# leohuang2013/pyannote-audio_speaker-diarization_cpp

Hardware: AMD Instinct MI355X
Metric: real-time factor (audio-sec/wall-sec), 1 h 16 kHz mono per GPU (higher is better)
Workload: dtype f32

## Files before the change

pyannote-audio_speaker-diarization_cpp_amd/csrc/api.cpp:

```cpp
#include "common.h"
#include <algorithm>
#include <cmath>
#include <cstdlib>
#include <fstream>
#include <tuple>

static std::string g_create_err;

int seg_prec(const sd_ctx* c) { return c->seg_precision >= 0 ? c->seg_precision : (c->ecapa_precision != 0 ? 3 : 0); }

extern "C" const char* sd_create_error(void) { return g_create_err.c_str(); }
extern "C" const char* sd_last_error(const sd_ctx* c) { return c ? c->err.c_str() : "null context"; }

extern "C" sd_ctx* sd_create(const char* seg_path, const char* emb_path, int device)
{
    g_create_err.clear();
    int ndev = 0;
    if (hipGetDeviceCount(&ndev) != hipSuccess || ndev <= 0) { g_create_err = "no HIP device available (libsdhip has no CPU fallback)"; return nullptr; }
    if (device < 0 || device >= ndev) { g_create_err = "device id out of range"; return nullptr; }
    if (hipSetDevice(device) != hipSuccess) { g_create_err = "hipSetDevice failed"; return nullptr; }
    sd_ctx* c = new sd_ctx();
    c->device = device;
    hipDeviceProp_t prop;
    if (hipGetDeviceProperties(&prop, device) == hipSuccess) c->num_cu = prop.multiProcessorCount;
// ... 46 lines not shown
    }
    c->pending.clear();
}

extern "C" int sd_kernel_stats(const sd_ctx* cc, const char* kernel, double* total_ms, int64_t* launches, double* flops, double* bytes)
{
    sd_ctx* c = const_cast<sd_ctx*>(cc);
    if (!c || !kernel) return SD_ERR_ARG;
    (void)hipStreamSynchronize(c->stream);
    sd_flush_profile(c);
    auto it = c->stats.find(kernel);
    KernelStat s; if (it != c->stats.end()) s = it->second;
    if (total_ms) *total_ms = s.ms; if (launches) *launches = s.launches; if (flops) *flops = s.flops; if (bytes) *bytes = s.bytes;
    return SD_OK;
}
extern "C" int sd_debug_read_ws(sd_ctx* c, const char* name, int64_t offset, void* h_out, int64_t bytes)
{
    if (!c || !name || !h_out || offset < 0 || bytes < 0) return SD_ERR_ARG;
    auto it = c->ws.find(name);
    if (it == c->ws.end() || !it->second.p) SD_FAIL(c, SD_ERR_ARG, "no workspace named %s", name);
    if ((size_t)(offset + bytes) > it->second.cap) SD_FAIL(c, SD_ERR_ARG, "workspace %s holds %zu bytes", name, it->second.cap);
    HIPCHK(c, hipStreamSynchronize(c->stream));
    HIPCHK(c, hipMemcpy(h_out, (const char*)it->second.p + offset, (size_t)bytes, hipMemcpyDeviceToHost));
    return SD_OK;
}
extern "C" void sd_reset_stats(sd_ctx* c) { if (!c) return; (void)hipStreamSynchronize(c->stream); sd_flush_profile(c); c->stats.clear(); }
extern "C" int sd_stage_ms(const sd_ctx* c, double* ms4) { if (!c || !ms4) return SD_ERR_ARG; for (int i = 0; i < 4; ++i) ms4[i] = c->stage_ms[i]; return SD_OK; }
extern "C" int sd_set_option(sd_ctx* c, const char* key, int64_t v)
{
    if (!c || !key) return SD_ERR_ARG;
    std::string k(key);
    if (k == "emb_batch_items") { c->emb_batch_items = v; c->emb_batch_explicit = true; }
    else if (k == "seg_batch_chunks") c->seg_batch_chunks = v;
    else if (k == "ws_limit_mb") g_ws_limit.store(v > 0 ? (size_t)v << 20 : 0);
    else if (k == "emb_batch_default") { c->emb_batch_items = 3072; c->emb_batch_explicit = false; c->embed_calls = v; }
    else if (k == "linkage_wgs") c->linkage_wgs = v;
    else if (k == "linkage_threads") c->linkage_threads = v;
    else if (k == "linkage_kernel") c->linkage_kernel = v;
    else if (k == "linkage_tie_kernel") c->linkage_tie_kernel = v;
    else if (k == "linkage_zero_phase") c->linkage_zero_phase = v;
    else if (k == "linkage_force_heap") c->linkage_force_heap = v != 0;
    else if (k == "linkage_hx_wide") c->linkage_hx_wide = v != 0;
    else if (k == "linkage_prefetch") c->linkage_prefetch = v != 0;
    else if (k == "linkage_one_xcd") c->linkage_one_xcd = v;
    else if (k == "linkage_square") c->linkage_square = v;
    else if (k == "skip_dead_rows") c->skip_dead_rows = v != 0;
    else if (k == "conv_h256") c->conv_h256 = v != 0;
    else if (k == "conv_glds") c->conv_glds = v != 0;
    else if (k == "conv_pp") c->conv_pp = v != 0;
    else if (k == "conv_glds_f32") c->conv_glds_f32 = v != 0;
    else if (k == "conv_mfma16") { if (v < 0 || v > 2) return SD_ERR_ARG; c->conv_mfma16 = (int)v; }
    else if (k == "conv_rot") { if (v < 0 || v > 3) return SD_ERR_ARG; c->conv_rot = (int)v; }
    else if (k == "conv_stagger") { if (v < 0 || v > 2) return SD_ERR_ARG; c->conv_stagger = (int)v; }
    else if (k == "conv_w256_f32") c->conv_w256_f32 = v != 0;
    else if (k == "conv_pn") c->conv_pn = (int)v;
    else if (k == "ecapa_ld_pad") { if (v < 0 || v > 1024 || ((int64_t)v & 7)) return SD_ERR_ARG; c->ecapa_ld_pad = (int)v; }
    else if (k == "seg_shared_conv0") c->seg_shared_conv0 = v != 0;
    else if (k == "seg_wide_ih") c->seg_wide_ih = v != 0;
    else if (k == "conv_w256_kmin") c->conv_w256_kmin = (int)v;
    else if (k == "conv_pn128") c->conv_pn128 = (int)v;
    else if (k == "seg_precision") { if (v != 0 && v != 3 && v != -1) SD_FAIL(c, SD_ERR_ARG, "seg_precision must be 0 (f32), 3 (split fp16 operands for the LSTM) or -1 (auto: 3 whenever ecapa_precision is not 0)"); c->seg_precision = (int)v; }
    else if (k == "ecapa_precision") { if (v < 0 || v > 3) SD_FAIL(c, SD_ERR_ARG, "ecapa_precision must be 0 (f32), 1 (fp16), 2 (fp16, hi + lo weight planes) or 3 (f32 tensors, split fp16 operands on the wide layers)");
                                        if (hipSetDevice(c->device) != hipSuccess) SD_FAIL(c, SD_ERR_HIP, "hipSetDevice failed");
                                        const int rcw = ensure_ecapa_mode_weights(c, (int)v); if (rcw) return rcw;
                                        c->ecapa_precision = (int)v; }
    else if (k == "ecapa_f16_hp") { if (v != 0 && v != 1 && v != 3) SD_FAIL(c, SD_ERR_ARG, "ecapa_f16_hp must be 0, 1 (MFA output in f32) or 3 (+ the attention branch)"); c->ecapa_f16_hp = (int)v; }
// ... 474 lines not shown
```

pyannote-audio_speaker-diarization_cpp_amd/csrc/common.h:

```cpp
#pragma once
#include <hip/hip_runtime.h>
#include <atomic>
#include <chrono>
#include <cstdint>
#include <cstdio>
#include <cstring>
#include <map>
#include <set>
#include <string>
#include <functional>
#include <initializer_list>
#include <vector>
#include "../../include/sdhip_test.h"

#define SD_T 501
#define SD_TP 501
#define SD_NBINS 201
#define SD_NMELS 80
#define SD_FEAT_LD 96

#define SD_WAV_PAD 512
struct DevWav {
    const float* p;
    int64_t n;
// ... 96 lines not shown
    void* lstm_hh_x[4][2] = {};
    float lstm_hh_inv[4][2] = {};
    ConvLayer lin0, lin1;
    float* cls_w = nullptr; float* cls_b = nullptr;
};

struct StepStash {
    bool clustered = false;
    int64_t N = 0; int K = 0;
    std::vector<int> clusters, cluster_res, hard_pre;
    std::vector<double> X, Xn, soft;
    int64_t ar0 = 0, cr0 = 0, rows = 0, crow_all = 0, nact = 0;
    int64_t infer_items = 0;
};

struct sd_ctx {
    int device = 0;
    hipStream_t stream = nullptr;
    std::string err;
    EcapaWeights ew;
    SegWeights sw;
    std::vector<void*> owned;
    char* warena_cur = nullptr; size_t warena_left = 0;
    std::map<std::string, DevBuf> ws;
    std::set<std::string> rs_taps_filled;
    std::map<std::string, KernelStat> stats;
    bool profile = false;
    bool profile_detail = false;
    std::vector<std::tuple<std::string, hipEvent_t, hipEvent_t, double, double>> pending;
    double stage_ms[4] = {0, 0, 0, 0};
    int64_t emb_batch_items = 3072;
    bool emb_batch_explicit = false;
    int64_t embed_calls = 0;
    int64_t seg_batch_chunks = 4096;
    int num_clusters = -1, min_clusters = -1, max_clusters = -1;
    int ecapa_precision = 0;
    int seg_precision = -1;
    bool ecapa_keep_cat = false;
    int ecapa_f16_hp = 0;
    bool conv_w256_f32 = true;
    int conv_pn128 = 0;
    int ecapa_ld_pad = 0;
    bool seg_wide_ih = true;
    bool seg_shared_conv0 = true;
    int conv_w256_kmin = 0;
    int conv_pn = 0;
    bool conv_h256 = true;
    int conv_mfma16 = 1;
    int conv_rot = 3;
    int conv_stagger = 0;
    bool conv_glds_f32 = false;
    bool conv_pp = true;
    bool conv_glds = true;
    bool skip_dead_rows = true;
    int64_t linkage_wgs = -1;
    int64_t linkage_square = -1;
    int64_t linkage_one_xcd = 1;
    int64_t linkage_zero_phase = 1;
    int64_t linkage_tie_kernel = 1;
    int64_t linkage_prefetch = 0;
    bool linkage_hx_wide = false;
    bool linkage_force_heap = false;
    int64_t linkage_kernel = -1;
    int64_t linkage_threads = 0;
    int num_cu = 256;
    bool constrained_assignment = false;
    int clustering_method = SD_LINKAGE_CENTROID;
// ... 107 lines not shown
float lstm_whh_split(const float* whh , _Float16* planes );
void* weight_alloc(sd_ctx* c, size_t bytes);
int ensure_ecapa_mode_weights(sd_ctx* c, int ecapa_precision);
inline size_t conv_w16_bytes(const ConvLayer& L) { return (size_t)2 * L.KT * L.Cout * L.CinPad16 * 2; }
inline size_t conv_w16x_bytes(const ConvLayer& L) { return (size_t)2 * L.KT * L.Cout * L.CinPad * 2; }
int build_conv_w16(sd_ctx* c, ConvLayer& L, void* d);
int build_conv_w16x(sd_ctx* c, ConvLayer& L, void* d, unsigned* d_max);
int frontend_prepare(sd_ctx* c, const float* d_masks, int64_t items, int64_t first_item, float* d_wav_lens, int* d_nnorm, int* d_nvalid,
                     int* d_flags, bool compact, int* h_n_active, int* d_cidx, std::vector<int>* h_nvalid = nullptr);
int frontend_features(sd_ctx* c, const DevWav& w, int64_t first_item, int64_t run_items, bool compact, const int* d_nnorm,
                      const int* d_rowoff, float* d_feats , bool sig_mode = false);
int frontend_prepare_signals(sd_ctx* c, int64_t items);
#define EC_SPACES 4
struct EcapaRowPlan {
    int64_t n = 0;
    std::vector<int> off[EC_SPACES];
    const int* d_off = nullptr;
};
int ecapa_need_rows(int nvalid, bool skip_dead_rows);
int ecapa_build_rowtab(sd_ctx* c, const int* d_off_out, int base_out, const int* d_off_in, int base_in, int64_t items, int2* d_rowtab);
int ecapa_rows_to_half(sd_ctx* c, const float* d_f32, void* d_f16, int64_t n4);
int ecapa_row_plan(sd_ctx* c, const int* h_nvalid, int64_t n, EcapaRowPlan& plan, int* d_off );
int run_ecapa(sd_ctx* c, const float* d_feats, const int* d_nvalid , const EcapaRowPlan& plan, int64_t a0, int64_t a1, float* d_emb );
std::vector<int64_t> ecapa_plan_batches(const EcapaRowPlan& plan, int64_t cap_rows, bool balance);
int64_t ecapa_round_items(int64_t nb);
int ecapa_run_items(sd_ctx* c, const float* d_feats, const int* d_nvalid, const EcapaRowPlan& plan, int64_t nb, bool balance, float* d_emb);
int run_embed(sd_ctx* c, const DevWav& w, const float* d_masks, int64_t items, int64_t first_item, float* d_emb);
int run_segment(sd_ctx* c, const DevWav& w, int64_t chunk_lo, int64_t chunk_hi, float* d_seg);
int run_segment_rows(sd_ctx* c, const DevWav& rows, int T, float* d_seg, int* frames);
int launch_chunk_norm(sd_ctx* c, const float* d_wav, int64_t origin, int64_t first_chunk, int64_t hop, int L, int64_t chunks, float w, float b, float* xn);
int launch_chunk_stats(sd_ctx* c, const float* d_wav, int64_t origin, int64_t first_chunk, int L, int64_t chunks, float w, float b, float2* st);
int launch_pool_norm(sd_ctx* c, int stage, const float* in, int64_t chunks, int Lc, const float* gw, const float* gb, float* out,
                     const float2* cst, const float* wsum, int chunk_rows);
int launch_lstm_rec(sd_ctx* c, const float* G, const float* whh_f, const float* whh_b, const void* whx_f, const void* whx_b, float inv_f, float inv_b,
                    float* H, int64_t B, int F);
int launch_classifier(sd_ctx* c, const float* y, const float* W, const float* bias, float* seg, int64_t chunks, int F);
__global__ void k_pcm_to_f32(const int16_t* __restrict__ pcm, float* __restrict__ dst, int64_t n);
int pcm_to_wav(sd_ctx* c, const int16_t* d_pcm, int64_t n, DevWav* out);
int f32_to_wav(sd_ctx* c, const float* h_wav, int64_t n, DevWav* out);
inline void clear_stage_ms(sd_ctx* c) { for (double& ms : c->stage_ms) ms = 0; }
int shard_infer(sd_ctx* c, const DevWav& w, int64_t lo, int64_t hi, float* d_seg, float* d_emb, bool seg_done = false);
int finalize(sd_ctx* c, const float* d_seg, const float* d_emb, int64_t chunks, int64_t n, std::vector<sd_turn>& v);
int turns_out(sd_ctx* c, const std::vector<sd_turn>& v, sd_turn** turns, int64_t* n_turns);
int resample_dev(sd_ctx* c, const float* d_in, int64_t n, int32_t in_sr, int32_t out_sr, float* d_out, int64_t n_out);
int run_postseg(sd_ctx* c, const float* d_seg, int64_t chunks, uint8_t* d_bin, float* d_masks, int* d_nact);
int run_count(sd_ctx* c, const uint8_t* d_bin, int64_t chunks, int32_t* d_count, int64_t n_count, double* d_avg = nullptr);
int write_step_dumps(sd_ctx* c, const float* d_seg, const float* d_emb, int64_t chunks, int64_t n_samples, const std::vector<int>& hard_post, int K);
int64_t count_frames_host(int64_t chunks);
int sd_np_rint_host(double v);
int64_t closest_frame_host(double w_start, double w_step, double w_dur, double t);
int run_linkage(sd_ctx* c, const double* d_X, int64_t N, int d, double* d_Z, int method = SD_LINKAGE_CENTROID, int metric = SD_METRIC_EUCLIDEAN);
int run_cluster_labels(sd_ctx* c, const double* d_X, int64_t N, int d, double cutoff, std::vector<int>& labels1, std::vector<double>* Zout = nullptr,
                       int method = SD_LINKAGE_CENTROID, int metric = SD_METRIC_EUCLIDEAN);
int run_clustering(sd_ctx* c, const double* d_emb , int64_t M, int d, std::vector<int>& hard, int* K,
                   int num_clusters = -1, int min_clusters = -1, int max_clusters = -1, std::vector<double>* soft_best = nullptr);
void fcluster_host(const std::vector<double>& Z, int64_t n, double cutoff, std::vector<int>& T);
int64_t activity_frames_host(int64_t chunks);
int64_t activity_rows_host(int64_t nf, int64_t n_samples);
int run_activity_scores(sd_ctx* c, const float* d_seg, int64_t chunks, int kind, double* d_scores, int64_t nf);
int run_activity_regions(sd_ctx* c, const double* d_scores, int64_t rows, int label, std::vector<sd_turn>& turns);
int check_spans(sd_ctx* c, const sd_turn* spans, int64_t n_spans, const char* who);
void spans_to_samples(const sd_turn* spans, int64_t n_spans, int32_t label, int64_t n, std::vector<int64_t>& out);
int run_span_masks(sd_ctx* c, const std::vector<int64_t>& spans, int64_t chunks, int64_t n, float* d_masks );
int run_voiceprint_mean(sd_ctx* c, const float* d_emb , int64_t chunks, double* h_mean , int64_t* n_live);
int run_speaker_dist(sd_ctx* c, const double* d_cen, int64_t K, const double* d_gal, int64_t M, int d, double* d_dist, double* h_dist );
int run_reconstruct(sd_ctx* c, const float* d_seg, const int* d_nact, const int* d_hard, const int32_t* d_count,
// ... 2 lines not shown
```

pyannote-audio_speaker-diarization_cpp_amd/csrc/pyannet.hip:

```cpp
#include "common.h"

typedef float f32x16 __attribute__((ext_vector_type(16)));

__global__ __launch_bounds__(256) void k_chunk_norm(const float* __restrict__ wav, int64_t origin, int64_t first_chunk, int64_t hop, int L,
                                                    float w, float b, float* __restrict__ xn)
{
    __shared__ float red[256];
    const int ck = blockIdx.x, tid = threadIdx.x;
    const int64_t base = (first_chunk + ck) * hop - origin;
    const float* x = wav + base;
    float s = 0.0f;
    for (int j = tid; j < L; j += 256) s += x[j];
    red[tid] = s;
    __syncthreads();
    for (int o = 128; o > 0; o >>= 1) { if (tid < o) red[tid] += red[tid + o]; __syncthreads(); }
    const float mean = red[0] / (float)L;
    __syncthreads();
    float v = 0.0f;
    for (int j = tid; j < L; j += 256) { const float d = x[j] - mean; v += d * d; }
    red[tid] = v;
    __syncthreads();
    for (int o = 128; o > 0; o >>= 1) { if (tid < o) red[tid] += red[tid + o]; __syncthreads(); }
    const float rstd = rsqrtf(red[0] / (float)L + 1e-5f);
    const float a = rstd * w, c = b - mean * rstd * w;
// ... 241 lines not shown
        const float giv[8] = {gi[0].x, gi[0].y, gi[0].z, gi[0].w, gi[1].x, gi[1].y, gi[1].z, gi[1].w};
        const float gfv[8] = {gf[0].x, gf[0].y, gf[0].z, gf[0].w, gf[1].x, gf[1].y, gf[1].z, gf[1].w};
        const float ggv[8] = {gg[0].x, gg[0].y, gg[0].z, gg[0].w, gg[1].x, gg[1].y, gg[1].z, gg[1].w};
        const float gov[8] = {go[0].x, go[0].y, go[0].z, go[0].w, go[1].x, go[1].y, go[1].z, go[1].w};
        float hv[8];
#pragma unroll
        for (int r = 0; r < 8; ++r) {
            const float ig = sigm(acc0[r] * inv + giv[r]);
            const float fg = sigm(acc0[r + 8] * inv + gfv[r]);
            const float gt = tanh_fast(acc1[r] * inv + ggv[r]);
            const float og = sigm(acc1[r + 8] * inv + gov[r]);
            cst[r] = fg * cst[r] + ig * gt;
            hv[r] = og * tanh_fast(cst[r]);
        }
        _Float16* hn = &hbuf[cur ^ 1][li * HXLD];
        lhalf4 h0, l0, h1, l1;
#pragma unroll
        for (int e = 0; e < 4; ++e) {
            h0[e] = (_Float16)hv[e];     l0[e] = (_Float16)(hv[e] - (float)h0[e]);
            h1[e] = (_Float16)hv[4 + e]; l1[e] = (_Float16)(hv[4 + e] - (float)h1[e]);
        }
        *(lhalf4*)(hn + ua) = h0; *(lhalf4*)(hn + 128 + ua) = l0;
        *(lhalf4*)(hn + ub) = h1; *(lhalf4*)(hn + 128 + ub) = l1;
        if (live) {
            float* ho = H + ((size_t)(b0 + li) * F + t) * 256 + dir * 128;
            *(float4*)(ho + ua) = make_float4(hv[0], hv[1], hv[2], hv[3]);
            *(float4*)(ho + ub) = make_float4(hv[4], hv[5], hv[6], hv[7]);
        }
        __syncthreads();
        cur ^= 1;
    }
}

__global__ __launch_bounds__(256) void k_classifier(const float* __restrict__ y, const float* __restrict__ W, const float* __restrict__ bias,
                                                    float* __restrict__ seg, int64_t chunks, int F)
{
    __shared__ float w[3 * 128];
    for (int i = threadIdx.x; i < 384; i += 256) w[i] = W[i];
    __syncthreads();
    const int64_t idx = (int64_t)blockIdx.x * 256 + threadIdx.x;
    if (idx >= chunks * SD_FRAMES) return;
    const int64_t ck = idx / SD_FRAMES;
    const int f = (int)(idx - ck * SD_FRAMES);
    float o0 = 0.0f, o1 = 0.0f, o2 = 0.0f;
    if (f < F) {
        const float* x = y + ((size_t)ck * F + f) * 128;
        float a0 = bias[0], a1 = bias[1], a2 = bias[2];
        for (int k = 0; k < 128; k += 4) {
            const float4 v = *(const float4*)(x + k);
            a0 += v.x * w[k] + v.y * w[k + 1] + v.z * w[k + 2] + v.w * w[k + 3];
            a1 += v.x * w[128 + k] + v.y * w[129 + k] + v.z * w[130 + k] + v.w * w[131 + k];
            a2 += v.x * w[256 + k] + v.y * w[257 + k] + v.z * w[258 + k] + v.w * w[259 + k];
        }
        o0 = 1.0f / (1.0f + expf(-a0)); o1 = 1.0f / (1.0f + expf(-a1)); o2 = 1.0f / (1.0f + expf(-a2));
    }
    seg[idx * 3 + 0] = o0; seg[idx * 3 + 1] = o1; seg[idx * 3 + 2] = o2;
}

__global__ void k_zero_f32(float* p, int64_t n)
{
    const int64_t i = (int64_t)blockIdx.x * blockDim.x + threadIdx.x;
    if (i < n) p[i] = 0.0f;
}

__global__ void k_dense_rowtab(int2* __restrict__ rowtab, int64_t M)
{
// ... 2 lines not shown
}

int launch_chunk_norm(sd_ctx* c, const float* d_wav, int64_t origin, int64_t first_chunk, int64_t hop, int L, int64_t chunks, float w, float b, float* xn)
{
    hipLaunchKernelGGL(k_chunk_norm, dim3((unsigned)chunks), dim3(256), 0, c->stream, d_wav, origin, first_chunk, hop, L, w, b, xn);
    KCHECK(c);
    return SD_OK;
}

int launch_chunk_stats(sd_ctx* c, const float* d_wav, int64_t origin, int64_t first_chunk, int L, int64_t chunks, float w, float b, float2* st)
{
    hipLaunchKernelGGL(k_chunk_stats, dim3((unsigned)chunks), dim3(256), 0, c->stream, d_wav, origin, first_chunk, L, w, b, st);
    KCHECK(c);
    return SD_OK;
}

int launch_pool_norm(sd_ctx* c, int stage, const float* in, int64_t chunks, int Lc, const float* gw, const float* gb, float* out,
                     const float2* cst, const float* wsum, int chunk_rows)
{
    const int Lp = Lc / 3;
    const dim3 grid((unsigned)chunks), block(PN_T);
    if (stage == 0 && cst)
        hipLaunchKernelGGL((k_pool_norm<80, 96, true, true>), grid, block, 0, c->stream, in, Lc, Lp, gw, gb, out, cst, wsum, chunk_rows);
    else if (stage == 0)
        hipLaunchKernelGGL((k_pool_norm<80, 96, true, false>), grid, block, 0, c->stream, in, Lc, Lp, gw, gb, out, nullptr, nullptr, 0);
    else if ((stage == 1 || stage == 2) && !cst)
        hipLaunchKernelGGL((k_pool_norm<60, 64, false, false>), grid, block, 0, c->stream, in, Lc, Lp, gw, gb, out, nullptr, nullptr, 0);
    else
        SD_FAIL(c, SD_ERR_ARG, "k_pool_norm: stage %d%s", stage, cst ? " (shared form)" : "");
    KCHECK(c);
    return SD_OK;
}

int launch_lstm_rec(sd_ctx* c, const float* G, const float* whh_f, const float* whh_b, const void* whx_f, const void* whx_b, float inv_f, float inv_b,
                    float* H, int64_t B, int F)
{
    ProfScope ps(c, "lstm_rec", 2.0 * B * F * 2 * 512 * 128, 0);
    const dim3 grid((unsigned)((B + 31) / 32), 2), block(512);
    if (whx_f && whx_b)
        hipLaunchKernelGGL(k_lstm_rec_x3, grid, block, 0, c->stream, G, (const _Float16*)whx_f, (const _Float16*)whx_b, inv_f, inv_b, H, (int)B, F);
    else
        hipLaunchKernelGGL(k_lstm_rec, grid, block, 0, c->stream, G, whh_f, whh_b, H, (int)B, F);
    KCHECK(c);
    return SD_OK;
}

int launch_classifier(sd_ctx* c, const float* y, const float* W, const float* bias, float* seg, int64_t chunks, int F)
{
    hipLaunchKernelGGL(k_classifier, GRID1(chunks * SD_FRAMES), 0, c->stream, y, W, bias, seg, chunks, F);
    KCHECK(c);
    return SD_OK;
}

static ConvArgs gemm_args(const ConvLayer& L, const float* X, int x_ld, float* Y, int y_ld, int64_t M)
{
    ConvArgs a;
    memset(&a, 0, sizeof(a));
    a.X = X; a.x_ld = x_ld; a.Y = Y; a.y_ld = y_ld; a.W = L.W; a.bias = L.bias;
    a.M = (int)M; a.TpIn = a.TpOut = (int)M; a.Tin = a.T = (int)M;
    a.Cin = L.CinPad; a.cin_real = L.Cin; a.Cout = L.Cout; a.KT = L.KT; a.dil = L.dil; a.pad_mode = 1;
    return a;
}

static int seg_batch(sd_ctx* c, const DevWav& w, int64_t first_chunk, int64_t cnt, int L, float* d_seg, int64_t hop = SD_HOP)
{
    const SegWeights& S = c->sw;
    hipStream_t st = c->stream;
    const int L0 = (L >= 251) ? (L - 251) / 10 + 1 : 0;
    const int P0 = L0 / 3, L1 = P0 - 4, P1 = L1 / 3, L2 = P1 - 4, P2 = L2 / 3;
    if (L0 <= 0 || P0 <= 0 || L1 <= 0 || P1 <= 0 || L2 <= 0 || P2 <= 0) {
        hipLaunchKernelGGL(k_zero_f32, GRID1(cnt * SD_FRAMES * 3), 0, st, d_seg, cnt * SD_FRAMES * 3);
        KCHECK(c);
// ... 33 lines not shown
            ConvArgs a; memset(&a, 0, sizeof(a));
            a.X = xn; a.x_ld = 10; a.W = S.conv0.W; a.Y = c0; a.y_ld = 80;
            a.M = (int)(CB * L0); a.TpIn = SD_CHUNK / 10; a.TpOut = L0; a.Tin = SD_CHUNK / 10; a.T = L0;
            a.Cin = 256; a.cin_real = 251; a.Cout = 80; a.KT = 1; a.dil = 1; a.pad_mode = 1;
            if ((rc = launch_conv_narrow(c, a, "sinc0")) == 1) rc = launch_conv_gemm(c, a, "sinc0");
            if (rc) return rc;
        }
        if ((rc = launch_pool_norm(c, 0, c0, CB, L0, S.in_w[0], S.in_b[0], p0, nullptr, nullptr, 0))) return rc;
    }
    {
        ConvArgs a; memset(&a, 0, sizeof(a));
        a.X = p0; a.x_ld = 96; a.W = S.conv1.W; a.bias = S.conv1.bias; a.Y = c1; a.y_ld = 60;
        a.M = (int)(CB * L1); a.TpIn = P0; a.TpOut = L1; a.Tin = P0; a.T = L1;
        a.Cin = 96; a.cin_real = 80; a.Cout = 60; a.KT = 5; a.dil = 1; a.pad_mode = 1;
        if ((rc = launch_conv_narrow(c, a, "sinc1")) == 1) rc = launch_conv_gemm(c, a, "sinc1");
        if (rc) return rc;
    }
    if ((rc = launch_pool_norm(c, 1, c1, CB, L1, S.in_w[1], S.in_b[1], p1, nullptr, nullptr, 0))) return rc;
    {
        ConvArgs a; memset(&a, 0, sizeof(a));
        a.X = p1; a.x_ld = 64; a.W = S.conv2.W; a.bias = S.conv2.bias; a.Y = c2; a.y_ld = 60;
        a.M = (int)(CB * L2); a.TpIn = P1; a.TpOut = L2; a.Tin = P1; a.T = L2;
        a.Cin = 64; a.cin_real = 60; a.Cout = 60; a.KT = 5; a.dil = 1; a.pad_mode = 1;
        if ((rc = launch_conv_narrow(c, a, "sinc2")) == 1) rc = launch_conv_gemm(c, a, "sinc2");
        if (rc) return rc;
    }
    if ((rc = launch_pool_norm(c, 2, c2, CB, L2, S.in_w[2], S.in_b[2], p2, nullptr, nullptr, 0))) return rc;
    const float* lin = p2; int lin_ld = 64; int lin_rows_per_chunk = P2;
    float* hout = Ha;
    int2* dense_tab = nullptr;
    for (int l = 0; l < 4; ++l) {
        if (lin_rows_per_chunk != F) SD_FAIL(c, SD_ERR_ARG, "unexpected frame count %d", P2);
        {
            ConvArgs a = gemm_args(S.lstm_ih[l], lin, lin_ld, G, 1024, CB * F);
            if (c->seg_wide_ih && l > 0 && CB * F <= (int64_t)ROWTAB_MAX_ITEMS * 512) {
                if (!dense_tab) {
                    dense_tab = ws_get<int2>(c, "seg_dense_rowtab", (size_t)(CB * F) + 512);
                    if (!dense_tab) SD_FAIL(c, SD_ERR_HIP, "hipMalloc of the dense row table failed");
                    hipLaunchKernelGGL(k_dense_rowtab, dim3((unsigned)((CB * F + 255) / 256)), dim3(256), 0, st, dense_tab, CB * F);
                    KCHECK(c);
                }
                a.rowtab = dense_tab; a.pad_mode = 0; a.Tin = 512; a.T = 512; a.TpIn = a.TpOut = 512; a.in_rows = (int)(CB * F);
                if (seg_prec(c) == 3 && S.lstm_ih[l].W16x) { a.prec = 3; a.W16x = S.lstm_ih[l].W16x; a.acc_scale = S.lstm_ih[l].w16x_inv; }
            }
            if ((rc = launch_conv_gemm(c, a, "lstm_ih"))) return rc;
        }
        {
            const bool x3 = seg_prec(c) == 3 && S.lstm_hh_x[l][0] && S.lstm_hh_x[l][1];
            if ((rc = launch_lstm_rec(c, G, S.lstm_hh[l][0], S.lstm_hh[l][1], x3 ? S.lstm_hh_x[l][0] : nullptr, x3 ? S.lstm_hh_x[l][1] : nullptr,
                                      S.lstm_hh_inv[l][0], S.lstm_hh_inv[l][1], hout, CB, F))) return rc;
        }
        lin = hout; lin_ld = 256; lin_rows_per_chunk = F;
        hout = (hout == Ha) ? Hb : Ha;
    }
    { ConvArgs a = gemm_args(S.lin0, lin, 256, y0, 128, CB * F); a.act1 = 2; if ((rc = launch_conv_gemm(c, a, "lin0"))) return rc; }
    { ConvArgs a = gemm_args(S.lin1, y0, 128, y1, 128, CB * F); a.act1 = 2; if ((rc = launch_conv_gemm(c, a, "lin1"))) return rc; }
    return launch_classifier(c, y1, S.cls_w, S.cls_b, d_seg, CB, F);
}

int run_segment(sd_ctx* c, const DevWav& w, int64_t chunk_lo, int64_t chunk_hi, float* d_seg)
{
    if (!c->sw.loaded) SD_FAIL(c, SD_ERR_MODEL, "segmentation model not loaded");
    int64_t last_len = 0;
    const int64_t total = sd_num_chunks(w.n, &last_len);
    if (chunk_lo < 0 || chunk_hi > total || chunk_lo > chunk_hi) SD_FAIL(c, SD_ERR_ARG, "chunk range [%lld,%lld) outside [0,%lld)", (long long)chunk_lo, (long long)chunk_hi, (long long)total);
    int64_t full_hi = chunk_hi;
    const bool has_short_tail = (chunk_hi == total) && (last_len > 0) && (last_len < SD_CHUNK);
    if (has_short_tail) full_hi = total - 1;
    int64_t cb = c->seg_batch_chunks;
    if (cb < 1) cb = 1;
    int rc;
    for (int64_t k = chunk_lo; k < full_hi; k += cb) {
        const int64_t cnt = (full_hi - k < cb) ? full_hi - k : cb;
        if ((rc = seg_batch(c, w, k, cnt, SD_CHUNK, d_seg + (size_t)(k - chunk_lo) * SD_FRAMES * 3))) return rc;
    }
    if (has_short_tail && chunk_lo <= total - 1)
        if ((rc = seg_batch(c, w, total - 1, 1, (int)last_len, d_seg + (size_t)(total - 1 - chunk_lo) * SD_FRAMES * 3))) return rc;
    return SD_OK;
// ... 18 lines not shown
```

pyannote-audio_speaker-diarization_cpp_amd/sdhip.py:

```python
import ctypes as C
import os
import numpy as np

_HERE = os.path.dirname(os.path.abspath(__file__))
LIB_PATH = os.environ.get("SDHIP_LIB") or os.path.join(_HERE, "libsdhip.so")

CHUNK, HOP, FRAMES, SPEAKERS, EMB_DIM, EMB_BATCH = 80000, 8000, 293, 3, 192, 32
T_FRAMES, N_MELS = 501, 80


class Turn(C.Structure):
    _fields_ = [("start", C.c_double), ("end", C.c_double), ("label", C.c_int32), ("_pad", C.c_int32)]


class ConvCase(C.Structure):
    _fields_ = [(n, C.c_int32) for n in (
        "items", "dense", "tin", "t", "tp_in", "tp_out", "cin", "cin_pad", "cout", "kt", "dil", "pad_mode",
        "shared", "x_ld", "x_col0", "has_x2", "x2_col0", "y_ld", "y_col0", "y_f32", "act1", "act2", "prec", "try_narrow")] + [("canary", C.c_float)]


CONV_SLACK_ROWS = 256
SEG_SLACK_ROWS = 256


# ... 116 lines not shown
    L.sd_stream_close.argtypes = [vp]
    L.sd_stream_close.restype = None
    L.sd_stream_sealed_chunks.restype = i64
    L.sd_stream_sealed_chunks.argtypes = [i64]
    L.sd_last_speakers.argtypes = [vp, vp, i64, C.POINTER(i64), vp]
    L.sd_span_masks.argtypes = [vp, i64, vp, i64, i32, vp]
    L.sd_voiceprint.argtypes = [vp, vp, i64, vp, i64, i32, vp, C.POINTER(i64)]
    L.sd_voiceprint_dev.argtypes = [vp, vp, i64, vp, i64, i32, vp, C.POINTER(i64)]
    L.sd_voiceprint_f32.argtypes = [vp, vp, i64, vp, i64, i32, vp, C.POINTER(i64)]
    L.sd_voiceprint_wav.argtypes = [vp, C.c_char_p, C.c_int, vp, i64, i32, vp, C.POINTER(i64)]
    L.sd_speaker_distances.argtypes = [vp, vp, i64, vp, i64, C.c_int, vp]
    L.sd_match_speakers.argtypes = [vp, vp, i64, vp, i64, C.c_int, dbl, vp, vp]
    L.sd_read_voiceprints.argtypes = [C.c_char_p, C.POINTER(C.POINTER(C.c_char_p)), C.POINTER(C.POINTER(dbl)), C.POINTER(i64)]
    L.sd_write_voiceprints.argtypes = [C.c_char_p, C.POINTER(C.c_char_p), vp, i64]
    L.sd_free_voiceprints.argtypes = [C.POINTER(C.c_char_p), C.POINTER(dbl), i64]
    L.sd_free_voiceprints.restype = None
    L.sd_voiceprints_error.restype = C.c_char_p
    L.sd_write_rttm_named.argtypes = [C.c_char_p, C.c_char_p, C.POINTER(Turn), i64, C.POINTER(dbl), C.POINTER(C.c_char_p), i64]
    L.sd_format_turn.argtypes = [C.POINTER(Turn), C.c_char_p, C.c_int]
    L.sd_stage_ms.argtypes = [vp, C.POINTER(dbl)]
    L.sd_kernel_stats.argtypes = [vp, C.c_char_p, C.POINTER(dbl), C.POINTER(i64), C.POINTER(dbl), C.POINTER(dbl)]
    L.sd_reset_stats.argtypes = [vp]
    L.sd_set_option.argtypes = [vp, C.c_char_p, i64]
    L.sd_convert_onnx.argtypes = [C.c_char_p, C.c_int, C.c_char_p]
    L.sd_convert_error.restype = C.c_char_p
    L.sd_debug_read_ws.argtypes = [vp, C.c_char_p, i64, vp, i64]
    L.sd_test_pack_split_weights.argtypes = [vp, C.c_int, C.c_int, C.c_int, C.c_int, vp, vp]
    L.sd_bench_conv.argtypes = [vp, i64] + [C.c_int] * 9 + [C.POINTER(dbl)]
    L.sd_test_conv.argtypes = [vp, C.POINTER(ConvCase)] + [vp] * 10 + [C.c_char_p, C.c_int]
    L.sd_test_lstm_rec.argtypes = [vp, vp, vp, vp, i64, C.c_int, C.c_int, C.c_float, vp]
    L.sd_test_pool_norm.argtypes = [vp, vp, i64, i64, C.c_int, C.c_int, vp, vp, vp, vp, C.c_int, C.c_float, vp]
    L.sd_test_chunk_norm.argtypes = [vp, vp, i64, i64, i64, i64, C.c_int, i64, C.c_float, C.c_float, C.c_int, C.c_float, vp]
    L.sd_test_classifier.argtypes = [vp, vp, vp, vp, i64, C.c_int, C.c_float, vp]
    L.sd_test_emb_batches.restype = i64
    L.sd_test_emb_batches.argtypes = [vp, i64, i64, C.c_int, C.c_int, vp, i64]
    _lib = L
    return L


def linkage_method_from_name(name):
    return int(lib().sd_linkage_method_from_name(str(name).encode()))


def _activity_kind(kind):
    if isinstance(kind, (int, np.integer)):
        return int(kind)
    return ACTIVITY_KINDS.index(kind) if kind in ACTIVITY_KINDS else -1


def _method_code(method):
    code = method if isinstance(method, (int, np.integer)) else linkage_method_from_name(method)
    return int(code)


def num_chunks(n):
    ll = C.c_int64(0)
    c = lib().sd_num_chunks(n, C.byref(ll))
    return int(c), int(ll.value)


def sealed_chunks(n):
    return int(lib().sd_stream_sealed_chunks(int(n)))


def fcluster(Z, cutoff):
    Z = np.ascontiguousarray(Z, np.float64).reshape(-1, 4)
    N = len(Z) + 1
    T = np.zeros(N, np.int32)
    rc = lib().sd_fcluster(None, _ptr(Z) if len(Z) else None, N, float(cutoff), _ptr(T))
    if rc:
        raise SdError(rc, "sd_fcluster: Z is not a dendrogram")
    return T


def emb_batches(nvalid, batch_items=3072, skip_dead_rows=True, balance=False):
    nv = np.ascontiguousarray(nvalid, np.int32)
    bounds = np.zeros(max(len(nv), 1), np.int64)
    nb = lib().sd_test_emb_batches(_ptr(nv), len(nv), int(batch_items), int(bool(skip_dead_rows)), int(bool(balance)), _ptr(bounds), len(bounds))
    if nb < 0:
        raise SdError(-nb, "sd_test_emb_batches: bad argument")
    return [int(b) for b in bounds[:nb]]


def shard_plan(n_total, world, rank0_permille=-1):
    arr = (C.c_int64 * (2 * world))()
    per = C.c_int64(0)
    rc = lib().sd_shard_plan(n_total, world, rank0_permille, arr, C.byref(per))
    if rc:
        raise SdError(rc, "sd_shard_plan: bad argument")
    return int(per.value), [(int(arr[2 * r]), int(arr[2 * r + 1])) for r in range(world)]


def plan_shards(n_total, world):
    return shard_plan(n_total, world, -1)


def plan_ranks(n_total, world, rank0_fraction=None):
    if rank0_fraction is None or world == 1:
        return shard_plan(n_total, world, -1)
    return shard_plan(n_total, world, int(round(1000.0 * max(0.0, min(1.0, rank0_fraction)))))


def gather_pieces(per, ranges):
    return [(r * per, hi - lo) for r, (lo, hi) in enumerate(ranges) if hi > lo]


def shard_sample_range(lo, hi, n_total):
    if hi <= lo:
        return lo * HOP, lo * HOP
    return lo * HOP, min(n_total, (hi - 1) * HOP + CHUNK)


def _ptr(a):
    return a.ctypes.data_as(C.c_void_p)
# ... 633 lines not shown
```

Baseline: 2956.

## Interleave two chunk sets per LSTM recurrence workgroup and double seg batch

Adds LSTM recurrence kernels where each workgroup handles two 32-chunk sets and alternates their matrix phase and gate phase, so one set's MFMA work can hide the other's elementwise and memory latency across the serial time loop. A planner selects this two-set form automatically when the grid would oversubscribe the CUs (f32 path only by default). The default seg_batch_chunks is doubled to 8192, and the input-hidden GEMM is split into parts so that larger batches fit the row-table limit. The trade-off is fewer workgroups and more barriers per step.

```diff
diff --git a/pyannote-audio_speaker-diarization_cpp_amd/csrc/api.cpp b/pyannote-audio_speaker-diarization_cpp_amd/csrc/api.cpp
--- a/pyannote-audio_speaker-diarization_cpp_amd/csrc/api.cpp
+++ b/pyannote-audio_speaker-diarization_cpp_amd/csrc/api.cpp
@@ -102,6 +102,7 @@
     std::string k(key);
     if (k == "emb_batch_items") { c->emb_batch_items = v; c->emb_batch_explicit = true; }
     else if (k == "seg_batch_chunks") c->seg_batch_chunks = v;
+    else if (k == "seg_lstm_form") { if (v < -1 || v > 1) SD_FAIL(c, SD_ERR_ARG, "seg_lstm_form must be -1 (auto), 0 (one chunk set per workgroup) or 1 (two)"); c->seg_lstm_form = (int)v; }
     else if (k == "ws_limit_mb") g_ws_limit.store(v > 0 ? (size_t)v << 20 : 0);
     else if (k == "emb_batch_default") { c->emb_batch_items = 3072; c->emb_batch_explicit = false; c->embed_calls = v; }
     else if (k == "linkage_wgs") c->linkage_wgs = v;
diff --git a/pyannote-audio_speaker-diarization_cpp_amd/csrc/common.h b/pyannote-audio_speaker-diarization_cpp_amd/csrc/common.h
--- a/pyannote-audio_speaker-diarization_cpp_amd/csrc/common.h
+++ b/pyannote-audio_speaker-diarization_cpp_amd/csrc/common.h
@@ -152,7 +152,8 @@
     int64_t emb_batch_items = 3072;
     bool emb_batch_explicit = false;
     int64_t embed_calls = 0;
-    int64_t seg_batch_chunks = 4096;
+    int64_t seg_batch_chunks = 8192;
+    int seg_lstm_form = -1;
     int num_clusters = -1, min_clusters = -1, max_clusters = -1;
     int ecapa_precision = 0;
     int seg_precision = -1;
@@ -326,6 +327,7 @@
 int launch_chunk_stats(sd_ctx* c, const float* d_wav, int64_t origin, int64_t first_chunk, int L, int64_t chunks, float w, float b, float2* st);
 int launch_pool_norm(sd_ctx* c, int stage, const float* in, int64_t chunks, int Lc, const float* gw, const float* gb, float* out,
                      const float2* cst, const float* wsum, int chunk_rows);
+int lstm_rec_plan(int64_t B, int num_cu, bool x3, int form_opt, unsigned* grid_x);
 int launch_lstm_rec(sd_ctx* c, const float* G, const float* whh_f, const float* whh_b, const void* whx_f, const void* whx_b, float inv_f, float inv_b,
                     float* H, int64_t B, int F);
 int launch_classifier(sd_ctx* c, const float* y, const float* W, const float* bias, float* seg, int64_t chunks, int F);
diff --git a/pyannote-audio_speaker-diarization_cpp_amd/csrc/pyannet.hip b/pyannote-audio_speaker-diarization_cpp_amd/csrc/pyannet.hip
--- a/pyannote-audio_speaker-diarization_cpp_amd/csrc/pyannet.hip
+++ b/pyannote-audio_speaker-diarization_cpp_amd/csrc/pyannet.hip
@@ -297,6 +297,232 @@
     }
 }
 
+__device__ __forceinline__ float tanh_fast_x(float x)
+{
+#pragma clang fp contract(off)
+    const float ax = fabsf(x), x2 = x * x;
+    const float small = x * __builtin_fmaf(x2, __builtin_fmaf(x2, __builtin_fmaf(x2, -0.053968254f, 0.13333334f), -0.33333334f), 1.0f);
+    const float big = copysignf(__builtin_fmaf(-2.0f, __builtin_amdgcn_rcpf(1.0f + __expf(2.0f * ax)), 1.0f), x);
+    return ax < 0.18f ? small : big;
+}
+__device__ __forceinline__ void lstm_cell_x(float pi, float pf, float pg, float po, float& c, float& og, float& th)
+{
+#pragma clang fp contract(off)
+    const float ig = sigm(pi), fg = sigm(pf), gt = tanh_fast_x(pg);
+    og = sigm(po);
+    c = __builtin_fmaf(ig, gt, fg * c);
+    th = tanh_fast_x(c);
+}
+
+__device__ __forceinline__ _Float16 h_lo_x(float h, float og, float th, _Float16 hi, bool fused)
+{
+#pragma clang fp contract(off)
+    return (_Float16)(fused ? __builtin_fmaf(og, th, -(float)hi) : h - (float)hi);
+}
+
+__global__ __launch_bounds__(512) void k_lstm_rec2(const float* __restrict__ G, const float* __restrict__ whh_f,
+                                                   const float* __restrict__ whh_b, float* __restrict__ H, int B, int F)
+{
+    __shared__ __attribute__((aligned(16))) float hbuf[2][2][32 * HLD];
+    const int dir = blockIdx.y, bA = blockIdx.x * 64, bB = bA + 32;
+    const int tid = threadIdx.x, lane = tid & 63, w = __builtin_amdgcn_readfirstlane(tid >> 6);
+    const int li = lane & 31, lh = lane >> 5;
+    const int u0 = 16 * w;
+    const bool grpY = w >= 4, haveB = bB < B;
+    const float* whh = dir ? whh_b : whh_f;
+
+    float A0[64], A1[64];
+    {
+        const int gsel = li >> 4, unit = u0 + (li & 15);
+        const float* r0 = whh + ((size_t)((0 + gsel) * 128 + unit)) * 128 + lh * 64;
+        const float* r1 = whh + ((size_t)((2 + gsel) * 128 + unit)) * 128 + lh * 64;
+#pragma unroll
+        for (int s = 0; s < 64; s += 4) {
+            const float4 v0 = *(const float4*)(r0 + s), v1 = *(const float4*)(r1 + s);
+            A0[s] = v0.x; A0[s + 1] = v0.y; A0[s + 2] = v0.z; A0[s + 3] = v0.w;
+            A1[s] = v1.x; A1[s + 1] = v1.y; A1[s + 2] = v1.z; A1[s + 3] = v1.w;
+        }
+    }
+    for (int i = tid; i < 2 * 2 * 32 * HLD; i += 512) (&hbuf[0][0][0])[i] = 0.0f;
+    float cstA[8], cstB[8];
+#pragma unroll
+    for (int r = 0; r < 8; ++r) { cstA[r] = 0.0f; cstB[r] = 0.0f; }
+    const int rowA = ((bA + li < B) ? (bA + li) : (B - 1)) * F, rowB = ((bB + li < B) ? (bB + li) : (B - 1)) * F;
+    const bool liveA = (bA + li) < B, liveB = (bB + li) < B;
+    const int ua = u0 + 4 * lh, ub = u0 + 8 + 4 * lh;
+    __syncthreads();
+
+    float4 gi[2], gf[2], gg[2], go[2];
+    f32x16 acc0, acc1;
+    auto slotM = [&](int row, int t, const float* hset) {
+        __builtin_amdgcn_s_setprio(1);
+        const float* g = G + (size_t)(row + t) * 1024 + dir * 512;
+        gi[0] = *(const float4*)(g + 0 * 128 + ua); gi[1] = *(const float4*)(g + 0 * 128 + ub);
+        gf[0] = *(const float4*)(g + 1 * 128 + ua); gf[1] = *(const float4*)(g + 1 * 128 + ub);
+        gg[0] = *(const float4*)(g + 2 * 128 + ua); gg[1] = *(const float4*)(g + 2 * 128 + ub);
+        go[0] = *(const float4*)(g + 3 * 128 + ua); go[1] = *(const float4*)(g + 3 * 128 + ub);
+#pragma unroll
+        for (int r = 0; r < 16; ++r) { acc0[r] = 0.0f; acc1[r] = 0.0f; }
+        const float* hb = hset + li * HLD + lh * 64;
+#pragma unroll
+        for (int s = 0; s < 64; s += 4) {
+            const float4 bv = *(const float4*)(hb + s);
+            acc0 = __builtin_amdgcn_mfma_f32_32x32x2f32(A0[s], bv.x, acc0, 0, 0, 0);
+            acc1 = __builtin_amdgcn_mfma_f32_32x32x2f32(A1[s], bv.x, acc1, 0, 0, 0);
+            acc0 = __builtin_amdgcn_mfma_f32_32x32x2f32(A0[s + 1], bv.y, acc0, 0, 0, 0);
+            acc1 = __builtin_amdgcn_mfma_f32_32x32x2f32(A1[s + 1], bv.y, acc1, 0, 0, 0);
+            acc0 = __builtin_amdgcn_mfma_f32_32x32x2f32(A0[s + 2], bv.z, acc0, 0, 0, 0);
+            acc1 = __builtin_amdgcn_mfma_f32_32x32x2f32(A1[s + 2], bv.z, acc1, 0, 0, 0);
+            acc0 = __builtin_amdgcn_mfma_f32_32x32x2f32(A0[s + 3], bv.w, acc0, 0, 0, 0);
+            acc1 = __builtin_amdgcn_mfma_f32_32x32x2f32(A1[s + 3], bv.w, acc1, 0, 0, 0);
+        }
+    };
+    auto slotG = [&](float (&cst)[8], float* hset, int row, bool live, int t) {
+        __builtin_amdgcn_s_setprio(0);
+        const float giv[8] = {gi[0].x, gi[0].y, gi[0].z, gi[0].w, gi[1].x, gi[1].y, gi[1].z, gi[1].w};
+        const float gfv[8] = {gf[0].x, gf[0].y, gf[0].z, gf[0].w, gf[1].x, gf[1].y, gf[1].z, gf[1].w};
+        const float ggv[8] = {gg[0].x, gg[0].y, gg[0].z, gg[0].w, gg[1].x, gg[1].y, gg[1].z, gg[1].w};
+        const float gov[8] = {go[0].x, go[0].y, go[0].z, go[0].w, go[1].x, go[1].y, go[1].z, go[1].w};
+        float hv[8];
+#pragma unroll
+        for (int r = 0; r < 8; ++r) {
+            float og, th;
+            lstm_cell_x(acc0[r] + giv[r], acc0[r + 8] + gfv[r], acc1[r] + ggv[r], acc1[r + 8] + gov[r], cst[r], og, th);
+            hv[r] = og * th;
+        }
+        float* hn = hset + li * HLD;
+        *(float4*)(hn + ua) = make_float4(hv[0], hv[1], hv[2], hv[3]);
+        *(float4*)(hn + ub) = make_float4(hv[4], hv[5], hv[6], hv[7]);
+        if (live) {
+            float* ho = H + (size_t)(row + t) * 256 + dir * 128;
+            *(float4*)(ho + ua) = make_float4(hv[0], hv[1], hv[2], hv[3]);
+            *(float4*)(ho + ub) = make_float4(hv[4], hv[5], hv[6], hv[7]);
+        }
+    };
+
+    if (grpY) __syncthreads();
+    int cur = 0;
+    for (int step = 0; step < F; ++step) {
+        const int t = dir ? (F - 1 - step) : step;
+        slotM(rowA, t, hbuf[0][cur]);
+        __syncthreads();
+        slotG(cstA, hbuf[0][cur ^ 1], rowA, liveA, t);
+        __syncthreads();
+        if (haveB) slotM(rowB, t, hbuf[1][cur]);
+        __syncthreads();
+        if (haveB) slotG(cstB, hbuf[1][cur ^ 1], rowB, liveB, t);
+        __syncthreads();
+        cur ^= 1;
+    }
+    if (!grpY) __syncthreads();
+}
+
+__global__ __launch_bounds__(512) void k_lstm_rec2_x3(const float* __restrict__ G, const _Float16* __restrict__ whh_f, const _Float16* __restrict__ whh_b,
+                                                      float inv_f, float inv_b, float* __restrict__ H, int B, int F)
+{
+    __shared__ __attribute__((aligned(16))) _Float16 hbuf[2][2][32 * HXLD];
+    const int dir = blockIdx.y, bA = blockIdx.x * 64, bB = bA + 32;
+    const int tid = threadIdx.x, lane = tid & 63, w = __builtin_amdgcn_readfirstlane(tid >> 6);
+    const int li = lane & 31, lh = lane >> 5;
+    const int u0 = 16 * w;
+    const bool grpY = w >= 4, haveB = bB < B;
+    const _Float16* whh = dir ? whh_b : whh_f;
+    const float inv = dir ? inv_b : inv_f;
+
+    lhalf8 Wr[2][2][8];
+    {
+        const int gsel = li >> 4, unit = u0 + (li & 15);
+#pragma unroll
+        for (int t = 0; t < 2; ++t)
+#pragma unroll
+            for (int pl = 0; pl < 2; ++pl)
+#pragma unroll
+                for (int kb = 0; kb < 8; ++kb)
+                    Wr[t][pl][kb] = *(const lhalf8*)(whh + (size_t)pl * 512 * 128 + ((size_t)((2 * t + gsel) * 128 + unit)) * 128 + 16 * kb + 8 * lh);
+    }
+    for (int i = tid; i < 2 * 2 * 32 * HXLD; i += 512) (&hbuf[0][0][0])[i] = (_Float16)0.0f;
+    float cstA[8], cstB[8];
+#pragma unroll
+    for (int r = 0; r < 8; ++r) { cstA[r] = 0.0f; cstB[r] = 0.0f; }
+    const int rowA = ((bA + li < B) ? (bA + li) : (B - 1)) * F, rowB = ((bB + li < B) ? (bB + li) : (B - 1)) * F;
+    const bool liveA = (bA + li) < B, liveB = (bB + li) < B;
+    const int ua = u0 + 4 * lh, ub = u0 + 8 + 4 * lh;
+    __syncthreads();
+
+    float4 gi[2], gf[2], gg[2], go[2];
+    auto fetch = [&](int row, int step) {
+        const int t = dir ? (F - 1 - step) : step;
+        const float* g = G + (size_t)(row + t) * 1024 + dir * 512;
+        gi[0] = *(const float4*)(g + 0 * 128 + ua); gi[1] = *(const float4*)(g + 0 * 128 + ub);
+        gf[0] = *(const float4*)(g + 1 * 128 + ua); gf[1] = *(const float4*)(g + 1 * 128 + ub);
+        gg[0] = *(const float4*)(g + 2 * 128 + ua); gg[1] = *(const float4*)(g + 2 * 128 + ub);
+        go[0] = *(const float4*)(g + 3 * 128 + ua); go[1] = *(const float4*)(g + 3 * 128 + ub);
+    };
+    f32x16 acc0, acc1;
+    auto slotM = [&](const _Float16* hset) {
+#pragma unroll
+        for (int r = 0; r < 16; ++r) { acc0[r] = 0.0f; acc1[r] = 0.0f; }
+        const _Float16* hb = hset + li * HXLD + 8 * lh;
+#pragma unroll
+        for (int kb = 0; kb < 8; ++kb) {
+            const lhalf8 hh = *(const lhalf8*)(hb + 16 * kb);
+            const lhalf8 hl = *(const lhalf8*)(hb + 128 + 16 * kb);
+            acc0 = __builtin_amdgcn_mfma_f32_32x32x16_f16(Wr[0][0][kb], hh, acc0, 0, 0, 0);
+            acc1 = __builtin_amdgcn_mfma_f32_32x32x16_f16(Wr[1][0][kb], hh, acc1, 0, 0, 0);
+            acc0 = __builtin_amdgcn_mfma_f32_32x32x16_f16(Wr[0][1][kb], hh, acc0, 0, 0, 0);
+            acc1 = __builtin_amdgcn_mfma_f32_32x32x16_f16(Wr[1][1][kb], hh, acc1, 0, 0, 0);
+            acc0 = __builtin_amdgcn_mfma_f32_32x32x16_f16(Wr[0][0][kb], hl, acc0, 0, 0, 0);
+            acc1 = __builtin_amdgcn_mfma_f32_32x32x16_f16(Wr[1][0][kb], hl, acc1, 0, 0, 0);
+        }
+    };
+    auto slotG = [&](float (&cst)[8], _Float16* hset, int row, bool live, int t, int nrow, int nstep) {
+        const float giv[8] = {gi[0].x, gi[0].y, gi[0].z, gi[0].w, gi[1].x, gi[1].y, gi[1].z, gi[1].w};
+        const float gfv[8] = {gf[0].x, gf[0].y, gf[0].z, gf[0].w, gf[1].x, gf[1].y, gf[1].z, gf[1].w};
+        const float ggv[8] = {gg[0].x, gg[0].y, gg[0].z, gg[0].w, gg[1].x, gg[1].y, gg[1].z, gg[1].w};
+        const float gov[8] = {go[0].x, go[0].y, go[0].z, go[0].w, go[1].x, go[1].y, go[1].z, go[1].w};
+        float hv[8], og[8], th[8];
+#pragma unroll
+        for (int r = 0; r < 8; ++r) {
+            lstm_cell_x(__builtin_fmaf(acc0[r], inv, giv[r]), __builtin_fmaf(acc0[r + 8], inv, gfv[r]), __builtin_fmaf(acc1[r], inv, ggv[r]),
+                        __builtin_fmaf(acc1[r + 8], inv, gov[r]), cst[r], og[r], th[r]);
+            hv[r] = og[r] * th[r];
+        }
+        fetch(nrow, nstep);
+        _Float16* hn = hset + li * HXLD;
+        lhalf4 h0, l0, h1, l1;
+#pragma unroll
+        for (int e = 0; e < 4; ++e) {
+            h0[e] = (_Float16)hv[e];     l0[e] = h_lo_x(hv[e], og[e], th[e], h0[e], e >= 2);
+            h1[e] = (_Float16)hv[4 + e]; l1[e] = h_lo_x(hv[4 + e], og[4 + e], th[4 + e], h1[e], e >= 2);
+        }
+        *(lhalf4*)(hn + ua) = h0; *(lhalf4*)(hn + 128 + ua) = l0;
+        *(lhalf4*)(hn + ub) = h1; *(lhalf4*)(hn + 128 + ub) = l1;
+        if (live) {
+            float* ho = H + (size_t)(row + t) * 256 + dir * 128;
+            *(float4*)(ho + ua) = make_float4(hv[0], hv[1], hv[2], hv[3]);
+            *(float4*)(ho + ub) = make_float4(hv[4], hv[5], hv[6], hv[7]);
+        }
+    };
+
+    fetch(rowA, 0);
+    if (grpY) __syncthreads();
+    int cur = 0;
+    for (int step = 0; step < F; ++step) {
+        const int t = dir ? (F - 1 - step) : step;
+        const int nxt = step + 1 < F ? step + 1 : step;
+        slotM(hbuf[0][cur]);
+        __syncthreads();
+        slotG(cstA, hbuf[0][cur ^ 1], rowA, liveA, t, haveB ? rowB : rowA, haveB ? step : nxt);
+        __syncthreads();
+        if (haveB) slotM(hbuf[1][cur]);
+        __syncthreads();
+        if (haveB) slotG(cstB, hbuf[1][cur ^ 1], rowB, liveB, t, rowA, nxt);
+        __syncthreads();
+        cur ^= 1;
+    }
+    if (!grpY) __syncthreads();
+}
+
 __global__ __launch_bounds__(256) void k_classifier(const float* __restrict__ y, const float* __restrict__ W, const float* __restrict__ bias,
                                                     float* __restrict__ seg, int64_t chunks, int F)
 {
@@ -365,12 +591,38 @@
     return SD_OK;
 }
 
+int lstm_rec_plan(int64_t B, int num_cu, bool x3, int form_opt, unsigned* grid_x)
+{
+    const int64_t sets = (B + 31) / 32;
+    const int form = form_opt == 0 ? 0 : form_opt == 1 ? 1 : (!x3 && 2 * sets > (int64_t)num_cu ? 1 : 0);
+    *grid_x = (unsigned)(form ? (sets + 1) / 2 : sets);
+    return form;
+}
+
+extern "C" int sd_test_lstm_plan(int64_t B, int num_cu, int prec, int form_opt, int64_t* grid_xy)
+{
+    if (B < 1 || num_cu < 1 || (prec != 0 && prec != 3) || form_opt < -1 || form_opt > 1 || !grid_xy) return -SD_ERR_ARG;
+    unsigned gx = 0;
+    const int form = lstm_rec_plan(B, num_cu, prec == 3, form_opt, &gx);
+    grid_xy[0] = gx; grid_xy[1] = 2;
+    return form;
+}
+
 int launch_lstm_rec(sd_ctx* c, const float* G, const float* whh_f, const float* whh_b, const void* whx_f, const void* whx_b, float inv_f, float inv_b,
                     float* H, int64_t B, int F)
 {
     ProfScope ps(c, "lstm_rec", 2.0 * B * F * 2 * 512 * 128, 0);
-    const dim3 grid((unsigned)((B + 31) / 32), 2), block(512);
-    if (whx_f && whx_b)
+    if (B < 1 || F < 1 || B * (int64_t)F > 0x7fffffff) SD_FAIL(c, SD_ERR_ARG, "lstm_rec: B %lld, F %d", (long long)B, F);
+    unsigned gx = 0;
+    const bool x3 = whx_f && whx_b;
+    const int form = lstm_rec_plan(B, c->num_cu, x3, c->seg_lstm_form, &gx);
+    const dim3 grid(gx, 2), block(512);
+    if (form) c->stats["lstm_rec_two_set"].launches += 1;
+    if (form && x3)
+        hipLaunchKernelGGL(k_lstm_rec2_x3, grid, block, 0, c->stream, G, (const _Float16*)whx_f, (const _Float16*)whx_b, inv_f, inv_b, H, (int)B, F);
+    else if (form)
+        hipLaunchKernelGGL(k_lstm_rec2, grid, block, 0, c->stream, G, whh_f, whh_b, H, (int)B, F);
+    else if (x3)
         hipLaunchKernelGGL(k_lstm_rec_x3, grid, block, 0, c->stream, G, (const _Float16*)whx_f, (const _Float16*)whx_b, inv_f, inv_b, H, (int)B, F);
     else
         hipLaunchKernelGGL(k_lstm_rec, grid, block, 0, c->stream, G, whh_f, whh_b, H, (int)B, F);
@@ -470,18 +722,24 @@
     for (int l = 0; l < 4; ++l) {
         if (lin_rows_per_chunk != F) SD_FAIL(c, SD_ERR_ARG, "unexpected frame count %d", P2);
         {
-            ConvArgs a = gemm_args(S.lstm_ih[l], lin, lin_ld, G, 1024, CB * F);
-            if (c->seg_wide_ih && l > 0 && CB * F <= (int64_t)ROWTAB_MAX_ITEMS * 512) {
-                if (!dense_tab) {
-                    dense_tab = ws_get<int2>(c, "seg_dense_rowtab", (size_t)(CB * F) + 512);
-                    if (!dense_tab) SD_FAIL(c, SD_ERR_HIP, "hipMalloc of the dense row table failed");
-                    hipLaunchKernelGGL(k_dense_rowtab, dim3((unsigned)((CB * F + 255) / 256)), dim3(256), 0, st, dense_tab, CB * F);
-                    KCHECK(c);
+            const int64_t rows = CB * F, span = (int64_t)ROWTAB_MAX_ITEMS * 512;
+            const int64_t parts = (c->seg_wide_ih && l > 0) ? (rows + span - 1) / span : 1;
+            const int64_t part = parts > 1 ? ((rows + parts - 1) / parts + 511) / 512 * 512 : rows;
+            for (int64_t r0 = 0; r0 < rows; r0 += part) {
+                const int64_t m = rows - r0 < part ? rows - r0 : part;
+                ConvArgs a = gemm_args(S.lstm_ih[l], lin + (size_t)r0 * lin_ld, lin_ld, G + (size_t)r0 * 1024, 1024, m);
+                if (c->seg_wide_ih && l > 0) {
+                    if (!dense_tab) {
+                        dense_tab = ws_get<int2>(c, "seg_dense_rowtab", (size_t)part + 512);
+                        if (!dense_tab) SD_FAIL(c, SD_ERR_HIP, "hipMalloc of the dense row table failed");
+                        hipLaunchKernelGGL(k_dense_rowtab, dim3((unsigned)((part + 255) / 256)), dim3(256), 0, st, dense_tab, part);
+                        KCHECK(c);
+                    }
+                    a.rowtab = dense_tab; a.pad_mode = 0; a.Tin = 512; a.T = 512; a.TpIn = a.TpOut = 512; a.in_rows = (int)m;
+                    if (seg_prec(c) == 3 && S.lstm_ih[l].W16x) { a.prec = 3; a.W16x = S.lstm_ih[l].W16x; a.acc_scale = S.lstm_ih[l].w16x_inv; }
                 }
-                a.rowtab = dense_tab; a.pad_mode = 0; a.Tin = 512; a.T = 512; a.TpIn = a.TpOut = 512; a.in_rows = (int)(CB * F);
-                if (seg_prec(c) == 3 && S.lstm_ih[l].W16x) { a.prec = 3; a.W16x = S.lstm_ih[l].W16x; a.acc_scale = S.lstm_ih[l].w16x_inv; }
+                if ((rc = launch_conv_gemm(c, a, "lstm_ih"))) return rc;
             }
-            if ((rc = launch_conv_gemm(c, a, "lstm_ih"))) return rc;
         }
         {
             const bool x3 = seg_prec(c) == 3 && S.lstm_hh_x[l][0] && S.lstm_hh_x[l][1];
diff --git a/pyannote-audio_speaker-diarization_cpp_amd/sdhip.py b/pyannote-audio_speaker-diarization_cpp_amd/sdhip.py
--- a/pyannote-audio_speaker-diarization_cpp_amd/sdhip.py
+++ b/pyannote-audio_speaker-diarization_cpp_amd/sdhip.py
@@ -172,6 +172,7 @@
     L.sd_test_pool_norm.argtypes = [vp, vp, i64, i64, C.c_int, C.c_int, vp, vp, vp, vp, C.c_int, C.c_float, vp]
     L.sd_test_chunk_norm.argtypes = [vp, vp, i64, i64, i64, i64, C.c_int, i64, C.c_float, C.c_float, C.c_int, C.c_float, vp]
     L.sd_test_classifier.argtypes = [vp, vp, vp, vp, i64, C.c_int, C.c_float, vp]
+    L.sd_test_lstm_plan.argtypes = [i64, C.c_int, C.c_int, C.c_int, vp]
     L.sd_test_emb_batches.restype = i64
     L.sd_test_emb_batches.argtypes = [vp, i64, i64, C.c_int, C.c_int, vp, i64]
     _lib = L
@@ -220,6 +221,14 @@
     if nb < 0:
         raise SdError(-nb, "sd_test_emb_batches: bad argument")
     return [int(b) for b in bounds[:nb]]
+
+
+def lstm_plan(B, num_cu=256, form=-1, prec=0):
+    g = np.zeros(2, np.int64)
+    f = lib().sd_test_lstm_plan(int(B), int(num_cu), int(prec), int(form), _ptr(g))
+    if f < 0:
+        raise SdError(-f, "sd_test_lstm_plan: bad argument")
+    return int(f), (int(g[0]), int(g[1]))
 
 
 def shard_plan(n_total, world, rank0_permille=-1):
```

Result: no change. 2967 (median of 6 runs) (+0.4%).
